# datatypevoid/babble

Hardware: AMD Instinct MI355X
Metric: consensus-ordered events/sec at N=256 peers (1 GPU and 8-GPU batched sims) (higher is better)
Workload: dtype int32

## Files before the change

babble_amd/_lib.py:

```python
from __future__ import annotations

import ctypes as C
import os

import numpy as np

HERE = os.path.dirname(os.path.abspath(__file__))
LIB_PATH = os.path.join(HERE, os.environ.get("HGX_LIB", "libhgx.so"))

_L = None


class HgxError(RuntimeError):

    def __init__(self, code: int, msg: str):
        super().__init__(msg)
        self.code = code
        self.msg = msg


class hgx_error(C.Structure):
    _fields_ = [("code", C.c_int32), ("msg", C.c_char * 252)]


# ... 146 lines not shown
    _sig(L, "hgx_get_block", i32, [p, i32, i32, p, E])
    _sig(L, "hgx_consensus_received", i32, [p, i32, i64, i64, p, p, p])
    _sig(L, "hgx_last_from", i32, [p, i32, p, p, E])
    _sig(L, "hgx_participant_events", i32, [p, i32, i64, p, i64, p, E])
    _sig(L, "hgx_participant_event", i32, [p, i32, i64, p, E])
    _sig(L, "hgx_get_root", i32, [p, i32, p, p, p, p, E])
    _sig(L, "hgx_get_event", i32, [p, i64, p, p, p, p, p, p, p, E])
    _sig(L, "hgx_wire_info", i32, [p, i64, i64, p, p, p])
    _sig(L, "hgx_read_wire_info", i32, [p, i32, i64, i32, i64, p, p, E])
    _sig(L, "hgx_diff_wire", i32, [p, i32, p, i64, p, i64, C.POINTER(C.c_int64), C.POINTER(C.c_int32), E])
    _sig(L, "hgx_keep_bodies", i32, [p, i64, i64, E])
    _sig(L, "hgx_bodies_state", i32, [p, C.POINTER(C.c_int64), C.POINTER(C.c_int64), C.POINTER(C.c_int64)])
    _sig(L, "hgx_get_event_bodies", i32, [p, p, i64, p, p, p, i64, p, i64, C.POINTER(C.c_int64),
                                          C.POINTER(C.c_int64), E])
    _sig(L, "hgx_block_transactions", i32, [p, i32, i64, p, i64, p, i64, C.POINTER(C.c_int64),
                                            C.POINTER(C.c_int64), E])
    _sig(L, "hgx_get_block_hash", i32, [p, i32, i64, p, E])
    _sig(L, "hgx_block_hash_batch", i32, [i32, p, p, p, p, p, i64, p, E])
    _sig(L, "hgx_diff_wire_bodies", i32, [p, i32, p, i64, p, C.POINTER(hgx_wire_body_out), i64, C.POINTER(C.c_int64),
                                          C.POINTER(C.c_int64), C.POINTER(C.c_int64), C.POINTER(C.c_int32), E])
    _sig(L, "hgx_get_rounds", i32, [p, i64, i64, p, p, p])
    _sig(L, "hgx_get_received", i32, [p, i64, i64, p, p])
    _sig(L, "hgx_get_coords", i32, [p, i64, p, p])
    for nm in ("hgx_ancestor", "hgx_self_ancestor", "hgx_see", "hgx_strongly_see", "hgx_round", "hgx_witness"):
        _sig(L, nm, i32, [p, i64, i64] if nm not in ("hgx_round", "hgx_witness") else [p, i64])
    _sig(L, "hgx_oldest_self_ancestor_to_see", i64, [p, i64, i64])
    _sig(L, "hgx_block_hash", i32, [i64, i32, p, p, i32, p])
    _sig(L, "hgx_sha256_batch", i32, [i32, p, p, i64, p, p])
    _sig(L, "hgx_sha256_batch_device", i32, [p, p, i64, p, p])
    _sig(L, "hgx_p256_verify_batch", i32, [i32, p, i32, p, p, p, p, i64, p, p])
    _sig(L, "hgx_p256_verify_bench", i32, [i32, p, i32, p, p, p, p, i64, i32, i32, p, C.POINTER(C.c_double)])
    _sig(L, "hgx_sha256_bench", i32, [i32, i64, i32, i32, C.c_uint64, i32, i32, C.POINTER(C.c_double),
                                      C.POINTER(C.c_int64), C.POINTER(C.c_int64), i64, p])
    _sig(L, "hgx_phase_times", i32, [p, p, i32])
    _sig(L, "hgx_kernel_stats", i32, [p, i32, C.c_char_p, i32, C.POINTER(C.c_double), C.POINTER(C.c_int64),
                                      C.POINTER(C.c_double)])
    _sig(L, "hgx_reset_stats", i32, [p])
    _sig(L, "hgx_set_kernel_timing", i32, [p, i32])
    _sig(L, "hgx_set_coord_storage", i32, [p, i32])
    _sig(L, "hgx_set_fame_tally", i32, [p, i32])
    _sig(L, "hgx_set_round_kernel", i32, [p, i32])
    _sig(L, "hgx_set_sort_kernel", i32, [p, i32])
    _sig(L, "hgx_set_round_shards", i32, [p, i32])
    _sig(L, "hgx_set_shard_remote", i32, [p, i32])
    _sig(L, "hgx_exchange_floor_bench", i32, [i32, i32, i32, i32, C.POINTER(C.c_double)])
    _sig(L, "hgx_seg_sort_check", i32, [i32, i32, p, i32, p, p, p, i32, p, C.POINTER(C.c_int32)])
# ... 32 lines not shown
```

babble_amd/csrc/hgx_api.cpp:

```cpp
#include <algorithm>
#include <array>
#include <chrono>
#include <cstdio>
#include <cstring>
#include <mutex>
#include <tuple>
#include <set>
#include <new>
#include <cstdlib>
#include <string>
#include <thread>
#include <vector>

#include "hgx.h"
#include "hgx_bodies.h"
#include "hgx_bodystore.h"
#include "hgx_diff.h"
#include "hgx_engine.h"
#include "hgx_wire_plan.h"

namespace {

struct Block {
    int32_t rr;
// ... 2691 lines not shown
    }
    return HGX_OK;
}

int32_t hgx_get_received(hgx_ctx* c, int64_t first, int64_t count, int32_t* rr, int64_t* cts) {
    if (!c || first < 0 || count < 0 || first + count > c->E) return HGX_ERR_INVALID;
    DeviceGuard dg(c);
    if (ensure_received(c)) return HGX_ERR_DEVICE;
    for (int64_t k = 0; k < count; k++) {
        const size_t x = (size_t)(first + k);
        const bool have = x < c->rr_cache.size();
        if (rr) rr[k] = have ? c->rr_cache[x] : -1;
        if (cts) cts[k] = (have && c->rr_cache[x] >= 0) ? c->cts_cache[x] : 0;
    }
    return HGX_OK;
}

int32_t hgx_get_coords(hgx_ctx* c, int64_t gid, int32_t* la, int32_t* fd) {
    if (!c || gid < 0 || gid >= c->E_div || !c->divided) return HGX_ERR_INVALID;
    DeviceGuard dg(c);
    return c->eng.get_coords(gid, la, fd) == hipSuccess ? HGX_OK : HGX_ERR_DEVICE;
}

static bool known_div(hgx_ctx* c, int64_t x) { return c && x >= 0 && x < c->E_div && c->divided; }
static bool same_graph(hgx_ctx* c, int64_t x, int64_t y) { return graph_of(c, x) == graph_of(c, y); }

int32_t hgx_ancestor(hgx_ctx* c, int64_t x, int64_t y) {
    if (x == y) return 1;
    if (!known_div(c, x) || !known_div(c, y)) return 0;
    DeviceGuard dg(c);
    if (ensure_mirror(c) || !same_graph(c, x, y)) return 0;
    std::vector<int32_t> la(c->n), fd(c->n);
    if (c->eng.get_coords(x, la.data(), fd.data()) != hipSuccess) return 0;
    return la[c->creator[(size_t)y] % c->n] >= c->index32[(size_t)y] ? 1 : 0;
}
int32_t hgx_self_ancestor(hgx_ctx* c, int64_t x, int64_t y) {
    if (x == y) return 1;
    if (!c || x < 0 || y < 0 || x >= c->E || y >= c->E) return 0;
    DeviceGuard dg(c);
    if (ensure_mirror(c)) return 0;
    return (c->creator[(size_t)x] == c->creator[(size_t)y] && c->index32[(size_t)x] >= c->index32[(size_t)y]) ? 1 : 0;
}
int32_t hgx_see(hgx_ctx* c, int64_t x, int64_t y) { return hgx_ancestor(c, x, y); }
int32_t hgx_strongly_see(hgx_ctx* c, int64_t x, int64_t y) {
    if (!known_div(c, x) || !known_div(c, y)) return 0;
    DeviceGuard dg(c);
// ... 326 lines not shown
```

babble_amd/csrc/hgx_engine.cpp:

```cpp
#include "hgx_engine.h"
#include "hgx_bodystore.h"

#include <algorithm>
#include <array>
#include <chrono>
#include <cstdio>
#include <cstdlib>
#include <cstring>
#include <functional>

namespace hgx {

template <typename T>
hipError_t DBuf<T>::alloc(size_t count) {
    release();
    if (count == 0) count = 1;
    hipError_t e = hipMalloc((void**)&p, count * sizeof(T));
    if (e == hipSuccess) n = count; else p = nullptr;
    return e;
}

template <typename T>
hipError_t DBuf<T>::grow_copy(size_t count, size_t keep, hipStream_t s) {
    if (count <= n) return hipSuccess;
// ... 1297 lines not shown
    HGX_TRY(hipMemcpyAsync(ntx, g_ntx.p + gid, 4, hipMemcpyDeviceToHost, stream));
    HGX_TRY(hipMemcpyAsync(&nil, g_txnil.p + gid, 1, hipMemcpyDeviceToHost, stream));
    HGX_TRY(hipStreamSynchronize(stream));
    *tx_nil = nil;
    return hipSuccess;
}

hipError_t Engine::reserve_rounds(int32_t rounds) {
    rounds = std::max<int32_t>(rounds, 1);
    drop_step_graph();
    Bm.release(); WLA.release(); WFD.release(); wflag.release(); wstat.release(); wcoin.release();
    active.release(); Tthr.release(); fw.release(); elig.release(); ur_empty.release(); Smat.release();
    Vbuf.release(); fame.release(); blk_cnt.release(); blk_loaded.release(); blk_ntx.release(); blk_nil.release();
    ovf.release();
    WLAT.release();
    r_cap = 0;
    R = 0;
    E_div = 0;
    HGX_TRY(ensure_round_cap(rounds));
    return hipStreamSynchronize(stream);
}

int Engine::rebuild_segments(int64_t En, int coord_compact) const {
    if (G != 1 || En < (int64_t)kLaSegMinRows * C) return 1;
    const int cap_segs = (int)std::max<int64_t>(kLaMaxSegs, En / C / (2 * kLaHeadRows));
    return la_segs_override > 0 ? la_segs_override : la_wave_segments(n, coord_compact, num_cus, cap_segs);
}

void Engine::divide_rounds_rows(RoundsHost& out) {
    if (!rows_pending) return;
    rows_pending = false;
    for (size_t k = 0; k < rows_n && k < stage_out.size(); k++) {
        StagedD2H& d = stage_out[k];
        std::memcpy(d.dst, h_stage + d.off, d.bytes);
        d.bytes = 0;
    }
    out.bm.resize((size_t)(R + 1) * C);
    out.wflag.resize((size_t)R * C);
}

int32_t Engine::recv_round_lo(const RoundsHost& rh, int& max_unrecv) const {
    int32_t lo = R;
    max_unrecv = 0;
    if (E_div == 0 || rh.R == 0) return lo;
    for (int c = 0; c < C; c++) {
        const int32_t k = h_fu[c], len = h_len_div[c];
        if (k >= len) continue;
// ... 334 lines not shown

hipError_t Engine::get_coords(int64_t gid, int32_t* la, int32_t* fd) {
    int32_t pos = 0;
    HGX_TRY(hipMemcpyAsync(&pos, g_pos.p + gid, 4, hipMemcpyDeviceToHost, stream));
    HGX_TRY(hipStreamSynchronize(stream));
    if (!compact) {
        HGX_TRY(hipMemcpyAsync(la, LA.p + (size_t)pos * n, (size_t)n * 4, hipMemcpyDeviceToHost, stream));
        HGX_TRY(hipMemcpy2DAsync(fd, 4, FDT.p + pos, (size_t)fd_ld * 4, 4, (size_t)n, hipMemcpyDeviceToHost, stream));
        return hipStreamSynchronize(stream);
    }
    std::vector<uint16_t> l16(n), f16(n);
    const uint16_t* la16 = (const uint16_t*)LA.p;
    const uint16_t* fd16 = (const uint16_t*)FDT.p;
    HGX_TRY(hipMemcpyAsync(l16.data(), la16 + (size_t)pos * n, (size_t)n * 2, hipMemcpyDeviceToHost, stream));
    HGX_TRY(hipMemcpy2DAsync(f16.data(), 2, fd16 + pos, (size_t)fd_ld * 2, 2, (size_t)n, hipMemcpyDeviceToHost, stream));
    HGX_TRY(hipStreamSynchronize(stream));
    for (int i = 0; i < n; i++) {
        la[i] = (int32_t)l16[i] - 1;
        fd[i] = f16[i] == 0xFFFF ? 2147483647 : (int32_t)f16[i];
    }
    return hipSuccess;
}

}


namespace hgx {
void StepGraph::drop() {
    if (exec) (void)hipGraphExecDestroy(exec);
    if (graph) (void)hipGraphDestroy(graph);
    exec = nullptr;
    graph = nullptr;
}

void Engine::drop_step_graph() {
    for (auto& g : step_g) g.drop();
}
}
```

babble_amd/csrc/hgx_engine.h:

```cpp
#pragma once

#include <hip/hip_runtime.h>

#include <cstdint>
#include <string>
#include <atomic>
#include <condition_variable>
#include <mutex>
#include <thread>
#include <vector>

#include "hgx_divide_plan.h"
#include "hgx_ingest_cols.h"
#include "hgx_kernels.h"

#ifndef HGX_TRY
#define HGX_TRY(x)                              \
    do {                                        \
        hipError_t _e = (x);                    \
        if (_e != hipSuccess) return _e;        \
    } while (0)
#endif

namespace hgx {
// ... 223 lines not shown
    hipError_t find_order(const std::vector<uint8_t>& elig, const std::vector<uint8_t>& famous,
                          const std::vector<uint8_t>& ur_empty, int32_t r0, int max_unrecv, OrderHost& out);
    int32_t recv_round_lo(const RoundsHost& rh, int& max_unrecv) const;
    hipError_t find_order_begin(const std::vector<uint8_t>& elig, const std::vector<uint8_t>& famous,
                                const std::vector<uint8_t>& ur_empty, int32_t r0, int max_unrecv, OrderHost& out);
    hipError_t find_order_end(OrderHost& out, int32_t* order_dst = nullptr);
    int64_t shard_values(int lo, int hi) const;
    hipError_t shard_copy(int lo, int hi, void* buf, bool on_device, bool to_buf);
    int shard_lo = 0, shard_hi = 0;
    hipError_t set_roots(const std::vector<int32_t>& round, const std::vector<uint8_t>& y_ext);
    hipError_t set_root_others(const uint8_t* keys32, int64_t count);
    bool others_trust = false;
    bool rooted = false;
    int root_gmax = -1;
    hipError_t round_first_gids(int32_t r0, std::vector<int32_t>& out);
    hipError_t copy_order(int32_t* dst, int64_t first, int64_t count);
    hipError_t sync() { return hipStreamSynchronize(stream); }

    hipError_t reset_received();
    hipError_t reserve_rounds(int32_t rounds);
    hipError_t get_rounds(std::vector<int32_t>& round_by_gid);
    hipError_t get_received(std::vector<int32_t>& rr, std::vector<int64_t>& cts);
    hipError_t get_coords(int64_t gid, int32_t* la, int32_t* fd);

    int n = 0, G = 0, C = 0, sm = 0, nw = 1;
    int64_t cap = 0, E = 0, E_div = 0;
    int64_t Ppos = 0;
    bool incremental = true;
    bool last_rebuild = false;
    int32_t R = 0;
    int la_sweeps = 0;
    int la_kernel = 0;
    bool la_wave_used = false;
    int la_wave_segs = 1;
    int la_segs_override = 0;
    int num_cus = 256;
    static constexpr int kLaMaxSegs = 16;
    static constexpr int kLaHeadRows = 64;
    static constexpr int kLaSegMinRows = 512;
    int64_t la_wave_fallbacks = 0;
    bool la_verified = false;
    bool la_verify_always = false;
    int compact = 0;
    bool force_coord32 = false;
    int64_t la_rows = 0;
    static constexpr int kLaSeg = 16;
// ... 260 lines not shown
```

babble_amd/csrc/hgx_kernels.h:

```cpp
#pragma once

#include <hip/hip_runtime.h>

#include <cstdint>
#include <functional>
#include <vector>

namespace hgx {

constexpr int32_t kMaxI32 = 2147483647;
constexpr int32_t kWlatNotFamous = -2147483647 - 1;
constexpr int kOpkBits = 21;

struct DevArrays {
    const int32_t *g_creator, *g_index, *g_op, *g_ntx;
    const int64_t* g_ts;
    const uint8_t *g_S, *g_coin, *g_loaded, *g_txnil;
    int32_t *g_rr, *g_pos;
    int64_t* g_ck;
    int64_t* g_cts;
    const int32_t *c_off, *c_len, *c_base;
    int32_t *p_gid, *p_chain, *p_op, *p_opu, *p_round, *p_rr;
    int32_t* p_opk;
    int64_t *p_ts, *p_cts;
// ... 144 lines not shown
    int32_t* st[kMaxShards] = {};
    const void* FDT[kMaxShards] = {};
    int32_t c_split[kMaxShards + 1] = {};
};
hipError_t launch_xchg_floor(hipStream_t s, int C, int n, int rounds, uint32_t* rows, uint64_t* gran, int32_t* st);
hipError_t launch_round_p(hipStream_t s, const RoundArgs& A, uint32_t* FD8p, uint64_t* gran, int32_t* status,
                          int32_t* fin, int r0, int r_end, int init, int num_cus, int c_lo = 0, int c_hi = -1,
                          const RoundPWindows* win_dev = nullptr, int nwin = 1);
void launch_round_p_tail(hipStream_t s, const RoundArgs& A, const int32_t* fin, int r_last);
void launch_round_p_post(hipStream_t s, const RoundArgs& A, int r_lo, int r_hi);
bool round_pb_ok(int n, int G);
hipError_t launch_round_pb(hipStream_t s, const RoundArgs& A, uint32_t* FD8p, uint64_t* gran, int32_t* status,
                           int32_t* fin, const int32_t* amap, int na, int r0, int r_end, int num_cus, bool init);
void launch_round_pb_silent(hipStream_t s, const RoundArgs& A, int r_lo, int r_hi);
void launch_root_floor(hipStream_t s, const DevArrays& a, const int32_t* root_round, int32_t* gfl, int32_t* gB,
                       int gmax, int C, int n, int max_len);
void launch_round_first_gid(hipStream_t s, const DevArrays& a, int r0, int R, int C, int32_t* first);
void launch_last_round(hipStream_t s, int rs, int R, int G, int C, int n, const uint8_t* wstat, int32_t* lr);
void step_prof_dump();
void round_k_prof_dump();
void round_p_prof_dump();
void round_pb_prof_dump();
void round_g_prof_dump();
void launch_fame(hipStream_t s, const DevArrays& a, int r0, int R, int C, int n, int nw, int sm, int G, int tally);
void launch_wla_transpose(hipStream_t s, const DevArrays& a, int r0, int R, int G, int C, int n);
void launch_threshold(hipStream_t s, const DevArrays& a, int r0, int R, int C, int n);
void launch_round_received(hipStream_t s, const DevArrays& a, int R, int C, int n, int max_unrecv);
void launch_fu_advance(hipStream_t s, const DevArrays& a, int C);
void launch_fu_count(hipStream_t s, const DevArrays& a, int64_t E);
void launch_cts(hipStream_t s, const DevArrays& a, int c_lo, int c_cnt, int C, int n, int64_t P, int max_cnt);
bool cts_pipe_ok(int n, int C);
bool launch_cts_pipe(hipStream_t s, const DevArrays& a, int c_lo, int c_cnt, int C, int n, int64_t P, int max_cnt);
bool cts_row_ok(int n);
int cts_row_tile();
bool launch_cts_row(hipStream_t s, const DevArrays& a, int c_lo, int c_cnt, int C, int n, int64_t P, int max_cnt,
                    int R, int k_rows);
void launch_cts_shard_copy(hipStream_t s, const DevArrays& a, int lo, int hi, const int32_t* offs, int64_t* buf,
                           int to_buf);
void launch_minmax(hipStream_t s, const DevArrays& a, int32_t m);
void launch_sort(hipStream_t s, const DevArrays& a, int32_t m, int64_t cmin, int cts_bits, int R, int n,
                 int seg_bits, uint32_t** final_vals, uint64_t** final_keys);
int seg_sort_cap();
void launch_seg_count(hipStream_t s, const DevArrays& a, int32_t m, int R, int n, int nseg, uint32_t* segc,
                      unsigned long long* max_out);
hipError_t launch_sort_seg(hipStream_t s, const DevArrays& a, int32_t m, int64_t cmin, int cts_bits, int R, int n, int nseg,
                     uint32_t* segoff, uint32_t* segcur, int max_seg, uint32_t** final_vals, uint64_t** final_keys,
// ... 97 lines not shown
```

babble_amd/csrc/hgx_la_wave.hip:

```cpp
#include <hip/hip_runtime.h>

#include <algorithm>
#include <cstdint>

#include "hgx_device.h"
#include "hgx_kernels.h"

namespace hgx {

namespace {

template <typename CT>
struct LaW;
template <>
struct LaW<int32_t> {
    static constexpr uint32_t kNone = 0xFFFFFFFFu;
    __device__ __forceinline__ static uint32_t wmax(uint32_t a, uint32_t b) {
        return (uint32_t)max((int32_t)a, (int32_t)b);
    }
    static constexpr int kPerWord = 1;
    __device__ __forceinline__ static uint32_t own_mask(int) { return 0xFFFFFFFFu; }
    __device__ __forceinline__ static uint32_t own_bits(int, int32_t own) { return (uint32_t)own; }
};
template <>
struct LaW<uint16_t> {
    static constexpr uint32_t kNone = 0u;
    typedef unsigned short u16x2 __attribute__((ext_vector_type(2)));
    __device__ __forceinline__ static uint32_t wmax(uint32_t a, uint32_t b) {
        const u16x2 m = __builtin_elementwise_max(__builtin_bit_cast(u16x2, a), __builtin_bit_cast(u16x2, b));
        return __builtin_bit_cast(uint32_t, m);
    }
    static constexpr int kPerWord = 2;
    __device__ __forceinline__ static uint32_t own_mask(int cl) { return 0xFFFFu << ((cl & 1) * 16); }
    __device__ __forceinline__ static uint32_t own_bits(int cl, int32_t own) {
        return ((uint32_t)(own + 1) & 0xFFFFu) << ((cl & 1) * 16);
    }
};

#define HGX_CB() asm volatile("" ::: "memory")
__device__ __forceinline__ int32_t lds_ld(const int32_t* p) {
    HGX_CB();
    const int32_t v = *p;
    HGX_CB();
    return v;
}
__device__ __forceinline__ void lds_st(int32_t* p, int32_t v) {
    HGX_CB();
    *p = v;
    HGX_CB();
}

template <int DW>
__device__ __forceinline__ void settle(uint32_t (&v)[DW]) {
#pragma unroll
    for (int w = 0; w < DW; w++) asm volatile("" : "+v"(v[w]));
}

template <int DW>
__device__ __forceinline__ void ring_load(const uint32_t* p, uint32_t (&v)[DW]) {
// ... 16 lines not shown
    HGX_CB();
}
template <int DW>
__device__ __forceinline__ void ring_store(uint32_t* p, const uint32_t (&v)[DW]) {
    HGX_CB();
    if constexpr (DW % 8 == 0) {
#pragma unroll
        for (int k = 0; k < DW / 4; k++) ((uint4*)p)[k] = make_uint4(v[4 * k], v[4 * k + 1], v[4 * k + 2], v[4 * k + 3]);
    } else if constexpr (DW == 4) *(uint4*)p = make_uint4(v[0], v[1], v[2], v[3]);
    else if constexpr (DW == 2) *(uint2*)p = make_uint2(v[0], v[1]);
    else *p = v[0];
    HGX_CB();
}
template <int DW>
__device__ __forceinline__ void row_store(uint32_t* p, const uint32_t (&v)[DW]) {
    if constexpr (DW % 8 == 0) {
#pragma unroll
        for (int k = 0; k < DW / 4; k++) ((uint4*)p)[k] = make_uint4(v[4 * k], v[4 * k + 1], v[4 * k + 2], v[4 * k + 3]);
    } else if constexpr (DW == 4) *(uint4*)p = make_uint4(v[0], v[1], v[2], v[3]);
    else if constexpr (DW == 2) *(uint2*)p = make_uint2(v[0], v[1]);
    else *p = v[0];
}

constexpr int kTagEmpty = -1, kTagBusy = -2;
constexpr int kNoDesc = -2147483647 - 1;
constexpr uint32_t kSpinCap = 1u << 24;

}

__device__ __forceinline__ int chain_lower_bound(const int32_t* __restrict__ p_gid, int off, int len, int64_t x) {
    int lo = 0, hi = len;
    while (lo < hi) {
        const int mid = (lo + hi) >> 1;
        if ((int64_t)p_gid[off + mid] < x) lo = mid + 1;
        else hi = mid;
    }
    return lo;
}

template <typename CT, int DW, int R, int Q, int NLW, int J, int CH, int MODE>
__global__ void __launch_bounds__(1024) k_la_wave(uint32_t* __restrict__ LA, const int32_t* __restrict__ p_opk,
                                                  const int32_t* __restrict__ c_off, const int32_t* __restrict__ c_len,
                                                  const int32_t* __restrict__ c_base,
                                                  const int32_t* __restrict__ c_old,
                                                  const int32_t* __restrict__ p_gid, int64_t E, int nts, int head,
                                                  int n, int lgnp, int nwd, int nblk, int32_t* __restrict__ err,
                                                  const int32_t* __restrict__ lmap, int na, int ts0,
                                                  const int32_t* __restrict__ c_lim,
                                                  const int32_t* __restrict__ gate) {
    typedef LaW<CT> W;
    if (gate && *gate) return;
    extern __shared__ uint32_t smem[];
    const int NP = 1 << lgnp;
    uint32_t* ring_d = smem;
    int32_t* ring_t = (int32_t*)(ring_d + (size_t)R * NP * DW);
    int32_t* q = ring_t + R * NP;
    int32_t* lqv = q + Q * NP;
    int32_t* prog = lqv + n;
    int32_t* s_old = prog + n;
    int32_t* s_off = s_old + n;
    int32_t* s_len = s_off + n;
    int32_t* s_abort = s_len + n;
    const int b = blockIdx.x % nblk, ts = ts0 + (blockIdx.x / nblk) % nts, g = blockIdx.x / nblk / nts;
    const int c0 = g * n;
    const int wb = b * DW;
    const int tid = threadIdx.x;
    for (int t = tid; t < R * NP; t += blockDim.x) ring_t[t] = kTagEmpty;
    for (int t = tid; t < n; t += blockDim.x) {
        const int off = c_off[c0 + t], len = c_len[c0 + t];
        int o = 0, e = len;
        if constexpr (MODE == 1) o = c_old[c0 + t];
        if constexpr (MODE >= 2) {
            const int lim = c_lim ? c_lim[c0 + t] : len;
            o = ts == 0 ? 0 : chain_lower_bound(p_gid, off, lim, E * ts / nts);
            e = ts == nts - 1 ? lim : chain_lower_bound(p_gid, off, lim, E * (ts + 1) / nts);
            if constexpr (MODE == 3) e = ts == 0 ? o : min(e, o + head);
        }
        lqv[t] = o;
        prog[t] = o;
        s_old[t] = o;
        s_off[t] = off;
        s_len[t] = e;
    }
    if (tid == 0) *s_abort = 0;
    __syncthreads();
    const int nl = lmap ? na : n;
    const int ncw = (nl + 63) & ~63;
    if (tid >= ncw) {
        const int l = tid - ncw;
        uint32_t idle = 0;
// ... 2 lines not shown
            int lq[J];
#pragma unroll
            for (int j = 0; j < J; j++) {
                const int i = l + 64 * NLW * j;
                need[j] = false;
                lq[j] = 0;
                if (i < n) {
                    lq[j] = lds_ld(&lqv[i]);
                    if (lq[j] < s_len[i]) {
                        left = true;
                        need[j] = lq[j] + CH <= lds_ld(&prog[i]) + Q;
                    }
                }
            }
            if (!left) break;
            int32_t v[J][CH];
#pragma unroll
            for (int j = 0; j < J; j++)
                if (need[j]) {
                    const int i = l + 64 * NLW * j;
                    const int o = s_off[i] + lq[j], m = s_len[i] - lq[j];
#pragma unroll
                    for (int t = 0; t < CH; t++) v[j][t] = (t < m) ? p_opk[o + t] : -1;
                }
            bool any = false;
#pragma unroll
            for (int j = 0; j < J; j++)
                if (need[j]) {
                    const int i = l + 64 * NLW * j;
#pragma unroll
                    for (int t = 0; t < CH; t++) lds_st(&q[(((unsigned)(lq[j] + t) % Q) << lgnp) + i], v[j][t]);
                    HGX_CB();
                    lds_st(&lqv[i], min(lq[j] + CH, s_len[i]));
                    any = true;
                }
            if (any) {
                idle = 0;
            } else {
                if (lds_ld(s_abort) || ++idle > kSpinCap) break;
                __builtin_amdgcn_s_sleep(1);
            }
        }
        return;
    }
    if (tid >= nl) return;
    const int i = lmap ? lmap[tid] : tid;
    const int len = s_len[i];
    const int off = s_off[i];
    int own0 = c_base[c0 + i];
    asm volatile("" : "+v"(own0));
    const int ow = i / W::kPerWord - wb;
    const uint32_t omask = W::own_mask(i);
    int k = s_old[i];
    uint32_t carry[DW];
#pragma unroll
    for (int w = 0; w < DW; w++)
        carry[w] = (k > 0 && MODE != 2) ? LA[(size_t)(off + k - 1) * nwd + wb + w] : W::kNone;
    settle(carry);
    uint32_t* dst = LA + (size_t)(off + k) * nwd + wb;
    int opv = kNoDesc;
    uint32_t idle = 0;
    while (k < len) {
        const int lv = lds_ld(&lqv[i]);
        const int q0 = lds_ld(&q[(((unsigned)k % Q) << lgnp) + i]);
        const int q1 = lds_ld(&q[(((unsigned)(k + 1) % Q) << lgnp) + i]);
        const bool has_op = opv >= 0;
        const int opc = has_op ? (opv >> kOpkBits) : 0;
        const int opk = has_op ? (opv & ((1 << kOpkBits) - 1)) : 0;
        const int sl = (((unsigned)opk % R) << lgnp) + opc;
        int old = 0;
        int end = 0x7FFFFFFF;
        if constexpr (MODE != 0) old = lds_ld(&s_old[opc]);
        if constexpr (MODE == 3) end = lds_ld(&s_len[opc]);
        const int t1 = lds_ld(&ring_t[sl]);
        uint32_t od[DW];
        ring_load<DW>(ring_d + (size_t)sl * DW, od);
        const int t2 = lds_ld(&ring_t[sl]);
        bool ready = opv == -1 || (has_op && t1 == opk && t2 == opk);
        if (opv == -1) {
#pragma unroll
            for (int w = 0; w < DW; w++) od[w] = W::kNone;
        }
        const bool from_old = MODE != 0 && has_op && (opk < old || opk >= end);
        if (from_old || (has_op && !ready && t1 > opk)) {
            if (MODE == 2 && from_old) {
#pragma unroll
                for (int w = 0; w < DW; w++) od[w] = W::kNone;
            } else {
                uint32_t* src = LA + (size_t)(s_off[opc] + opk) * nwd + wb;
#pragma unroll
                for (int w = 0; w < DW; w++)
                    od[w] = __hip_atomic_load(src + w, __ATOMIC_RELAXED, __HIP_MEMORY_SCOPE_AGENT);
                settle(od);
            }
            ready = true;
        }
        const bool wave_idle = __ballot(ready) == 0;
        if (!ready) {
            if (opv == kNoDesc && lv > k) opv = q0;
            if (wave_idle) __builtin_amdgcn_s_sleep(1);
            if (((++idle) & 4095) == 0 && (idle > kSpinCap || lds_ld(s_abort))) {
                lds_st(s_abort, 1);
                atomicOr(err, 1);
                break;
            }
            continue;
        }
        idle = 0;
        uint32_t v[DW];
#pragma unroll
        for (int w = 0; w < DW; w++) {
            v[w] = W::wmax(carry[w], od[w]);
            v[w] = w == ow ? ((v[w] & ~omask) | W::own_bits(i, own0 + k)) : v[w];
        }
        if constexpr (DW == 16 && R == 8) asm volatile("s_waitcnt vmcnt(23)" ::: "memory");
        else if constexpr (R >= 16) asm volatile("s_waitcnt vmcnt(15)" ::: "memory");
        else asm volatile("s_waitcnt vmcnt(7)" ::: "memory");
        const int ws = (((unsigned)k % R) << lgnp) + i;
        lds_st(&ring_t[ws], kTagBusy);
        ring_store<DW>(ring_d + (size_t)ws * DW, v);
        lds_st(&ring_t[ws], k);
        row_store<DW>(dst, v);
        dst += nwd;
        lds_st(&prog[i], k + 1);
#pragma unroll
        for (int w = 0; w < DW; w++) carry[w] = v[w];
        k++;
        opv = lv > k ? q1 : kNoDesc;
    }
}

namespace {
template <typename CT, int DW, int R, int Q, int NLW, int J, int CH, int MODE>
hipError_t la_wave_launch1(hipStream_t s, const DevArrays& a, int G, int n, const int32_t* c_old, int64_t E, int nts,
                           int head, int32_t* err, const int32_t* lmap, int na, const LaSubset& sub = LaSubset()) {
    const int nwd = a.compact ? n / 2 : n;
    const int nblk = nwd / DW;
    int lgnp = 0;
    while ((1 << lgnp) < n) lgnp++;
    const size_t np2 = (size_t)1 << lgnp;
    const size_t words = np2 * (R * DW + R + Q) + 5 * (size_t)n + 1;
    auto kern = k_la_wave<CT, DW, R, Q, NLW, J, CH, MODE>;
    {
        const hipError_t e = ensure_lds_limit((const void*)kern, 160 * 1024);
        if (e != hipSuccess) return e;
    }
    const int threads = (((lmap ? na : n) + 63) & ~63) + 64 * NLW;
    if (threads > 1024 || (lmap && G != 1)) return hipErrorInvalidValue;
    const int nseg = sub.count > 0 ? sub.count : nts;
    hipLaunchKernelGGL(kern, dim3(G * nseg * nblk), dim3(threads), words * 4, s, (uint32_t*)a.LA, a.p_opk, a.c_off,
                       a.c_len, a.c_base, c_old, a.p_gid, E, nts, head, n, lgnp, nwd, nblk, err, lmap, na, sub.first,
                       sub.c_lim, sub.gate);
    return hipGetLastError();
}
template <typename CT, int DW, int R, int Q, int NLW, int J, int CH>
hipError_t la_wave_launch(hipStream_t s, const DevArrays& a, int G, int n, const int32_t* c_old, int64_t E,
                          int32_t* err, const int32_t* lmap, int na) {
    if (c_old) return la_wave_launch1<CT, DW, R, Q, NLW, J, CH, 1>(s, a, G, n, c_old, E, 1, 0, err, lmap, na);
    return la_wave_launch1<CT, DW, R, Q, NLW, J, CH, 0>(s, a, G, n, nullptr, E, 1, 0, err, lmap, na);
}
struct SegCfg {
    int dw, r, q;
};
inline SegCfg seg_cfg(int n, int nwd) {
// ... 181 lines not shown

hipError_t launch_la_small(hipStream_t s, const DevArrays& a, int G, int n, const int32_t* c_old, size_t lds,
                           int32_t* err) {
    switch (la_small_nw(a.compact ? n / 2 : n)) {
        case 1: return la_small_launch<1>(s, a, G, n, c_old, lds, err);
        case 2: return la_small_launch<2>(s, a, G, n, c_old, lds, err);
        case 4: return la_small_launch<4>(s, a, G, n, c_old, lds, err);
        case 8: return la_small_launch<8>(s, a, G, n, c_old, lds, err);
        case 16: return la_small_launch<16>(s, a, G, n, c_old, lds, err);
        default: return hipErrorInvalidValue;
    }
}

int la_wave_blocks(int n, int compact) {
    const int nwd = compact ? n / 2 : n;
    return nwd / seg_cfg(n, nwd).dw;
}

int la_wave_segments(int n, int compact, int num_cus, int max_segs) {
    const int nwd = compact ? n / 2 : n;
    const SegCfg g = seg_cfg(n, nwd);
    int np2 = 1;
    while (np2 < n) np2 <<= 1;
    const size_t bytes = ((size_t)np2 * (g.r * g.dw + g.r + g.q) + 5 * (size_t)n + 1) * 4;
    const int per_cu = std::max(1, std::min(4, (int)((160 * 1024) / bytes)));
    return std::max(1, std::min(max_segs, per_cu * num_cus / la_wave_blocks(n, compact)));
}

__global__ void __launch_bounds__(256) k_la_seg_bounds(const int32_t* __restrict__ p_gid, const int32_t* __restrict__ c_off,
                                                       const int32_t* __restrict__ c_len, int64_t E, int nts, int n,
                                                       int32_t* __restrict__ tbl) {
    const int t = blockIdx.x;
    for (int c = threadIdx.x; c < n; c += blockDim.x) {
        const int len = c_len[c];
        tbl[(size_t)t * n + c] = t == 0 ? 0 : t == nts ? len : chain_lower_bound(p_gid, c_off[c], len, E * t / nts);
    }
}

template <typename CT>
__global__ void __launch_bounds__(256) k_la_seg_check(const CT* __restrict__ LA, const int32_t* __restrict__ p_gid,
                                                      const int32_t* __restrict__ p_op, const int32_t* __restrict__ p_chain,
                                                      const int32_t* __restrict__ c_off, const int32_t* __restrict__ tbl,
                                                      int64_t E, int nts, int n, int head, int32_t* __restrict__ flag) {
    const int t = 1 + (int)blockIdx.x / n, c = (int)blockIdx.x % n;
    const int o = tbl[(size_t)t * n + c], e = tbl[(size_t)(t + 1) * n + c], off = c_off[c];
    bool bad = false;
    if (e - o > head) {
// ... 52 lines not shown
```

babble_amd/csrc/hgx_rounds.hip:

```cpp
#include <hip/hip_runtime.h>

#include <cstdint>
#include <cstdio>
#include <type_traits>
#include <utility>

#include "hgx_device.h"
#include "hgx_kernels.h"

namespace hgx {

#ifdef HGX_STEP_PROF
__device__ unsigned long long hgx_step_prof[8];
#define HGX_PROF_BEGIN() long long _pt = clock64(); unsigned long long _pa[8] = {0, 0, 0, 0, 0, 0, 0, 0}
#define HGX_PROF(i)                            \
    do {                                       \
        if (threadIdx.x == 0) {                \
            const long long _t = clock64();    \
            _pa[i] += (unsigned long long)(_t - _pt); \
            _pt = _t;                          \
        }                                      \
    } while (0)
#define HGX_PROF_COUNT(i) do { if (threadIdx.x == 0) _pa[i] += 1ull; } while (0)
#define HGX_PROF_END()                                                            \
// ... 638 lines not shown
    if (threadIdx.x == 0) {
        m = max(max(s_max[0], s_max[1]), max(s_max[2], s_max[3]));
        if (m >= 0) atomicMax(&lr[g], m);
    }
}

void launch_last_round(hipStream_t s, int rs, int R, int G, int C, int n, const uint8_t* wstat, int32_t* lr) {
    if (R <= rs) return;
    hipLaunchKernelGGL(k_last_round, dim3(G, (R - rs + 63) / 64), dim3(256), 0, s, rs, R, C, n, wstat, lr);
}


#ifdef HGX_STEP_PROF
void step_prof_dump() {
    unsigned long long h[8];
    if (hipMemcpyFromSymbol(h, HIP_SYMBOL(hgx_step_prof), sizeof(h)) != hipSuccess) return;
    fprintf(stderr, "[hgx] round phases (clk sums; 0 = block-rounds, 6 = wave-0 tallies*1000 + levels):");
    for (int i = 0; i < 8; i++) fprintf(stderr, " %d:%llu", i, h[i]);
    fprintf(stderr, "\n");
    round_k_prof_dump();
    round_p_prof_dump();
    round_pb_prof_dump();
    round_g_prof_dump();
}
#else
void step_prof_dump() {}
#endif

}
```

babble_amd/hashgraph.py:

```python
from __future__ import annotations

import ctypes as C
import os
from typing import List, Optional, Sequence

import numpy as np

from . import _lib
from ._lib import HgxError, hgx_error, hgx_events, ptr

UNKNOWN_PARENT = -2


def compact_columns(t) -> dict:
    ntx = np.where(np.asarray(t.txnil) != 0, -1, np.asarray(t.ntx)).astype(np.int32)
    return dict(creator=np.ascontiguousarray(t.creator, np.int32), index=np.ascontiguousarray(t.index, np.int32),
                sp=np.ascontiguousarray(t.sp, np.int32), op=np.ascontiguousarray(t.op, np.int32),
                ts=np.ascontiguousarray(t.ts, np.int64),
                coin=np.ascontiguousarray(np.asarray(t.hash)[:, 16] != 0, np.uint8),
                s=np.ascontiguousarray(t.s, np.uint8), ntx=ntx)


class HostBuffer:

# ... 766 lines not shown
    def See(self, x: int, y: int) -> bool:
        return bool(self.L.hgx_see(self.ctx, x, y))

    def StronglySee(self, x: int, y: int) -> bool:
        return bool(self.L.hgx_strongly_see(self.ctx, x, y))

    def OldestSelfAncestorToSee(self, x: int, y: int) -> int:
        return int(self.L.hgx_oldest_self_ancestor_to_see(self.ctx, x, y))

    def Round(self, x: int) -> int:
        return int(self.L.hgx_round(self.ctx, x))

    def Witness(self, x: int) -> bool:
        return bool(self.L.hgx_witness(self.ctx, x))

    def coords(self, x: int):
        la = np.zeros(self.n, np.int32)
        fd = np.zeros(self.n, np.int32)
        rc = self.L.hgx_get_coords(self.ctx, x, ptr(la), ptr(fd))
        if rc:
            raise HgxError(rc, "hgx_get_coords failed")
        return la, fd

    def num_events(self) -> int:
        return int(self.L.hgx_num_events(self.ctx))

    def rounds(self):
        E = self.num_events()
        rnd = np.zeros(max(E, 1), np.int32)
        wit = np.zeros(max(E, 1), np.int8)
        fam = np.zeros(max(E, 1), np.int8)
        if E:
            rc = self.L.hgx_get_rounds(self.ctx, 0, E, ptr(rnd), ptr(wit), ptr(fam))
            if rc:
                raise HgxError(rc, "hgx_get_rounds failed")
        return rnd[:E], wit[:E], fam[:E]

    def received(self):
        E = self.num_events()
        rr = np.zeros(max(E, 1), np.int32)
        cts = np.zeros(max(E, 1), np.int64)
        if E:
            rc = self.L.hgx_get_received(self.ctx, 0, E, ptr(rr), ptr(cts))
            if rc:
                raise HgxError(rc, "hgx_get_received failed")
        return rr[:E], cts[:E]
# ... 303 lines not shown
```

include/hgx.h:

```cpp
#ifndef HGX_H
#define HGX_H

#include <stdint.h>

#ifdef __cplusplus
extern "C" {
#endif

#define HGX_ABI_VERSION 6

enum {
    HGX_OK = 0,
    HGX_ERR_KEY_NOT_FOUND = 1,
    HGX_ERR_TOO_LATE = 2,
    HGX_ERR_PASSED_INDEX = 3,
    HGX_ERR_SKIPPED_INDEX = 4,
    HGX_ERR_NO_ROOT = 5,
    HGX_ERR_SELF_PARENT = 100,
    HGX_ERR_OTHER_PARENT = 101,
    HGX_ERR_INVALID = 102,
    HGX_ERR_CAPACITY = 103,
    HGX_ERR_SIGNATURE = 104,
    HGX_ERR_DEVICE = 200,
    HGX_ERR_PANIC = 300
// ... 230 lines not shown
                             int64_t* n_bytes, hgx_error* err);
int32_t hgx_block_transactions(hgx_ctx* ctx, int32_t graph, int64_t b, int64_t* tx_off, int64_t tx_cap,
                               uint8_t* tx_bytes, int64_t bytes_cap, int64_t* n_tx, int64_t* n_bytes, hgx_error* err);
int32_t hgx_get_block_hash(hgx_ctx* ctx, int32_t graph, int64_t b, uint8_t* out32, hgx_error* err);
int32_t hgx_block_hash_batch(int32_t device, const int64_t* round_received, const int32_t* ntx,
                             const int32_t* tx_nil, const int64_t* tx_off, const uint8_t* tx_bytes, int64_t count,
                             uint8_t* out32, hgx_error* err);
typedef struct {
    uint8_t* sig_r;
    int64_t* tx_off;
    int64_t tx_cap;
    uint8_t* tx_bytes;
    int64_t bytes_cap;
} hgx_wire_body_out;
int32_t hgx_diff_wire_bodies(hgx_ctx* ctx, int32_t graph, const int32_t* known, int64_t sync_limit,
                             hgx_wire_out* out, hgx_wire_body_out* body, int64_t cap, int64_t* count, int64_t* n_tx,
                             int64_t* n_bytes, int32_t* over_limit, hgx_error* err);

int32_t hgx_get_rounds(hgx_ctx* ctx, int64_t first, int64_t count, int32_t* round, int8_t* witness,
                       int8_t* famous);
int32_t hgx_get_received(hgx_ctx* ctx, int64_t first, int64_t count, int32_t* round_received,
                         int64_t* consensus_ts);
int32_t hgx_get_coords(hgx_ctx* ctx, int64_t gid, int32_t* last_ancestors, int32_t* first_descendants);

int32_t hgx_ancestor(hgx_ctx* ctx, int64_t x, int64_t y);
int32_t hgx_self_ancestor(hgx_ctx* ctx, int64_t x, int64_t y);
int32_t hgx_see(hgx_ctx* ctx, int64_t x, int64_t y);
int32_t hgx_strongly_see(hgx_ctx* ctx, int64_t x, int64_t y);
int64_t hgx_oldest_self_ancestor_to_see(hgx_ctx* ctx, int64_t x, int64_t y);
int32_t hgx_round(hgx_ctx* ctx, int64_t x);
int32_t hgx_witness(hgx_ctx* ctx, int64_t x);

int32_t hgx_block_hash(int64_t round_received, int32_t ntx, const uint8_t* const* tx, const int64_t* tx_len,
                       int32_t tx_nil, uint8_t* out32);

int32_t hgx_sha256_batch(int32_t device, const uint8_t* data, const int64_t* offsets, int64_t count,
                         uint8_t* out32, hgx_error* err);
int32_t hgx_sha256_batch_device(const uint8_t* d_data, const int64_t* d_offsets, int64_t count,
                                uint8_t* d_out32, void* stream);
int32_t hgx_sha256_bench(int32_t device, int64_t count, int32_t min_len, int32_t max_len, uint64_t seed,
                         int32_t warmup, int32_t iters, double* ms_per_launch, int64_t* total_bytes,
                         int64_t* n_blocks, int64_t n_sample, uint8_t* sample32);

int32_t hgx_exchange_floor_bench(int32_t device, int32_t chains, int32_t n, int32_t rounds, double* us_per_round);

int32_t hgx_seg_sort_check(int32_t device, int32_t nseg, const uint32_t* segoff, int32_t m, const uint64_t* keys,
// ... 47 lines not shown
```

Measured before the change: 288.5 million.

## Streamline LA wave loop: sentinel ring slot, sc1 row reads, mask-free owner merge

Reworks the last-ancestor wave kernel's inner loop. A sentinel ring slot replaces the branch for missing other-parents, and slot indices are now advanced incrementally instead of recomputed with modulos. Owner bits are merged through per-word masks with a wave-uniform guard, and read-backs use vectorised sc1 loads. In MODE 2, stale other-parent entries are filtered at queue fill time. Also adds a bulk coordinate read API, an optional profiler, and an override shortcut for segment count; these add LDS use and inline-asm coupling to the gfx950 ISA.

```diff
diff --git a/babble_amd/_lib.py b/babble_amd/_lib.py
--- a/babble_amd/_lib.py
+++ b/babble_amd/_lib.py
@@ -192,6 +192,7 @@
     _sig(L, "hgx_get_rounds", i32, [p, i64, i64, p, p, p])
     _sig(L, "hgx_get_received", i32, [p, i64, i64, p, p])
     _sig(L, "hgx_get_coords", i32, [p, i64, p, p])
+    _sig(L, "hgx_get_coords_range", i32, [p, i64, i64, p, p])
     for nm in ("hgx_ancestor", "hgx_self_ancestor", "hgx_see", "hgx_strongly_see", "hgx_round", "hgx_witness"):
         _sig(L, nm, i32, [p, i64, i64] if nm not in ("hgx_round", "hgx_witness") else [p, i64])
     _sig(L, "hgx_oldest_self_ancestor_to_see", i64, [p, i64, i64])
diff --git a/babble_amd/csrc/hgx_api.cpp b/babble_amd/csrc/hgx_api.cpp
--- a/babble_amd/csrc/hgx_api.cpp
+++ b/babble_amd/csrc/hgx_api.cpp
@@ -2737,6 +2737,13 @@
     return c->eng.get_coords(gid, la, fd) == hipSuccess ? HGX_OK : HGX_ERR_DEVICE;
 }
 
+int32_t hgx_get_coords_range(hgx_ctx* c, int64_t first, int64_t count, int32_t* la, int32_t* fd) {
+    if (!c || first < 0 || count < 0 || first + count > c->E_div || !c->divided || (count > 0 && (!la || !fd)))
+        return HGX_ERR_INVALID;
+    DeviceGuard dg(c);
+    return c->eng.get_coords_range(first, count, la, fd) == hipSuccess ? HGX_OK : HGX_ERR_DEVICE;
+}
+
 static bool known_div(hgx_ctx* c, int64_t x) { return c && x >= 0 && x < c->E_div && c->divided; }
 static bool same_graph(hgx_ctx* c, int64_t x, int64_t y) { return graph_of(c, x) == graph_of(c, y); }
 
diff --git a/babble_amd/csrc/hgx_engine.cpp b/babble_amd/csrc/hgx_engine.cpp
--- a/babble_amd/csrc/hgx_engine.cpp
+++ b/babble_amd/csrc/hgx_engine.cpp
@@ -1343,7 +1343,9 @@
 }
 
 int Engine::rebuild_segments(int64_t En, int coord_compact) const {
-    if (G != 1 || En < (int64_t)kLaSegMinRows * C) return 1;
+    if (G != 1) return 1;
+    if (la_segs_override > 0) return la_segs_override;
+    if (En < (int64_t)kLaSegMinRows * C) return 1;
     const int cap_segs = (int)std::max<int64_t>(kLaMaxSegs, En / C / (2 * kLaHeadRows));
     return la_segs_override > 0 ? la_segs_override : la_wave_segments(n, coord_compact, num_cus, cap_segs);
 }
@@ -1724,6 +1726,41 @@
     return hipSuccess;
 }
 
+hipError_t Engine::get_coords_range(int64_t first, int64_t count, int32_t* la, int32_t* fd) {
+    if (count <= 0) return hipSuccess;
+    std::vector<int32_t> pos((size_t)count);
+    HGX_TRY(hipMemcpyAsync(pos.data(), g_pos.p + first, (size_t)count * 4, hipMemcpyDeviceToHost, stream));
+    HGX_TRY(hipStreamSynchronize(stream));
+    const size_t hi = (size_t)*std::max_element(pos.begin(), pos.end()) + 1, csz = compact ? 2 : 4;
+    std::vector<uint8_t> lb(hi * n * csz), fb(hi * n * csz);
+    HGX_TRY(hipMemcpyAsync(lb.data(), LA.p, lb.size(), hipMemcpyDeviceToHost, stream));
+    HGX_TRY(hipMemcpy2DAsync(fb.data(), hi * csz, FDT.p, (size_t)fd_ld * csz, hi * csz, (size_t)n, hipMemcpyDeviceToHost,
+                             stream));
+    HGX_TRY(hipStreamSynchronize(stream));
+    for (int64_t x = 0; x < count; x++) {
+        const size_t p = (size_t)pos[(size_t)x];
+        int32_t* lo = la + (size_t)x * n;
+        int32_t* fo = fd + (size_t)x * n;
+        if (compact) {
+            const uint16_t* l16 = (const uint16_t*)lb.data() + p * n;
+            const uint16_t* f16 = (const uint16_t*)fb.data();
+            for (int i = 0; i < n; i++) {
+                lo[i] = (int32_t)l16[i] - 1;
+                const uint16_t f = f16[(size_t)i * hi + p];
+                fo[i] = f == 0xFFFF ? 2147483647 : (int32_t)f;
+            }
+        } else {
+            const int32_t* l32 = (const int32_t*)lb.data() + p * n;
+            const int32_t* f32 = (const int32_t*)fb.data();
+            for (int i = 0; i < n; i++) {
+                lo[i] = l32[i];
+                fo[i] = f32[(size_t)i * hi + p];
+            }
+        }
+    }
+    return hipSuccess;
+}
+
 }
 
 
diff --git a/babble_amd/csrc/hgx_engine.h b/babble_amd/csrc/hgx_engine.h
--- a/babble_amd/csrc/hgx_engine.h
+++ b/babble_amd/csrc/hgx_engine.h
@@ -269,6 +269,7 @@
     hipError_t get_rounds(std::vector<int32_t>& round_by_gid);
     hipError_t get_received(std::vector<int32_t>& rr, std::vector<int64_t>& cts);
     hipError_t get_coords(int64_t gid, int32_t* la, int32_t* fd);
+    hipError_t get_coords_range(int64_t first, int64_t count, int32_t* la, int32_t* fd);
 
     int n = 0, G = 0, C = 0, sm = 0, nw = 1;
     int64_t cap = 0, E = 0, E_div = 0;
diff --git a/babble_amd/csrc/hgx_kernels.h b/babble_amd/csrc/hgx_kernels.h
--- a/babble_amd/csrc/hgx_kernels.h
+++ b/babble_amd/csrc/hgx_kernels.h
@@ -190,6 +190,7 @@
 void round_p_prof_dump();
 void round_pb_prof_dump();
 void round_g_prof_dump();
+void la_wave_prof_dump();
 void launch_fame(hipStream_t s, const DevArrays& a, int r0, int R, int C, int n, int nw, int sm, int G, int tally);
 void launch_wla_transpose(hipStream_t s, const DevArrays& a, int r0, int R, int G, int C, int n);
 void launch_threshold(hipStream_t s, const DevArrays& a, int r0, int R, int C, int n);
diff --git a/babble_amd/csrc/hgx_la_wave.hip b/babble_amd/csrc/hgx_la_wave.hip
--- a/babble_amd/csrc/hgx_la_wave.hip
+++ b/babble_amd/csrc/hgx_la_wave.hip
@@ -2,6 +2,7 @@
 
 #include <algorithm>
 #include <cstdint>
+#include <cstdio>
 
 #include "hgx_device.h"
 #include "hgx_kernels.h"
@@ -21,6 +22,7 @@
     static constexpr int kPerWord = 1;
     __device__ __forceinline__ static uint32_t own_mask(int) { return 0xFFFFFFFFu; }
     __device__ __forceinline__ static uint32_t own_bits(int, int32_t own) { return (uint32_t)own; }
+    __device__ __forceinline__ static uint32_t own_word(uint32_t bits, uint32_t m) { return (bits & m) | ~m; }
 };
 template <>
 struct LaW<uint16_t> {
@@ -35,6 +37,7 @@
     __device__ __forceinline__ static uint32_t own_bits(int cl, int32_t own) {
         return ((uint32_t)(own + 1) & 0xFFFFu) << ((cl & 1) * 16);
     }
+    __device__ __forceinline__ static uint32_t own_word(uint32_t bits, uint32_t m) { return bits & m; }
 };
 
 #define HGX_CB() asm volatile("" ::: "memory")
@@ -97,11 +100,85 @@
     else *p = v[0];
 }
 
+template <int DW>
+__device__ __forceinline__ void row_load_sc1(const uint32_t* p, uint32_t (&v)[DW]) {
+    typedef uint32_t u32x4 __attribute__((ext_vector_type(4)));
+    if constexpr (DW == 16) {
+        u32x4 a, b, c, d;
+        asm volatile(
+            "global_load_dwordx4 %0, %4, off sc1\n\t"
+            "global_load_dwordx4 %1, %4, off offset:16 sc1\n\t"
+            "global_load_dwordx4 %2, %4, off offset:32 sc1\n\t"
+            "global_load_dwordx4 %3, %4, off offset:48 sc1\n\t"
+            "s_waitcnt vmcnt(0)"
+            : "=&v"(a), "=&v"(b), "=&v"(c), "=&v"(d) : "v"(p) : "memory");
+        const u32x4 q4[4] = {a, b, c, d};
+#pragma unroll
+        for (int k = 0; k < 4; k++) { v[4 * k] = q4[k].x; v[4 * k + 1] = q4[k].y; v[4 * k + 2] = q4[k].z; v[4 * k + 3] = q4[k].w; }
+    } else if constexpr (DW == 8) {
+        u32x4 a, b;
+        asm volatile(
+            "global_load_dwordx4 %0, %2, off sc1\n\t"
+            "global_load_dwordx4 %1, %2, off offset:16 sc1\n\t"
+            "s_waitcnt vmcnt(0)"
+            : "=&v"(a), "=&v"(b) : "v"(p) : "memory");
+        v[0] = a.x; v[1] = a.y; v[2] = a.z; v[3] = a.w; v[4] = b.x; v[5] = b.y; v[6] = b.z; v[7] = b.w;
+    } else if constexpr (DW == 4) {
+        u32x4 a;
+        asm volatile(
+            "global_load_dwordx4 %0, %1, off sc1\n\t"
+            "s_waitcnt vmcnt(0)"
+            : "=&v"(a) : "v"(p) : "memory");
+        v[0] = a.x; v[1] = a.y; v[2] = a.z; v[3] = a.w;
+    } else {
+#pragma unroll
+        for (int w = 0; w < DW; w++) v[w] = __hip_atomic_load(p + w, __ATOMIC_RELAXED, __HIP_MEMORY_SCOPE_AGENT);
+#pragma unroll
+        for (int w = 0; w < DW; w++) asm volatile("" : "+v"(v[w]));
+    }
+}
+
 constexpr int kTagEmpty = -1, kTagBusy = -2;
 constexpr int kNoDesc = -2147483647 - 1;
 constexpr uint32_t kSpinCap = 1u << 24;
 
-}
+#ifdef HGX_STEP_PROF
+constexpr int kLaProfWg = 4096, kLaProfN = 6;
+__device__ unsigned long long hgx_la_prof[4][kLaProfWg][kLaProfN];
+#define LA_PROF(...) __VA_ARGS__
+#else
+#define LA_PROF(...)
+#endif
+
+}
+
+#ifdef HGX_STEP_PROF
+void la_wave_prof_dump() {
+    static unsigned long long h[4][kLaProfWg][kLaProfN];
+    if (hipMemcpyFromSymbol(h, HIP_SYMBOL(hgx_la_prof), sizeof(h)) != hipSuccess) return;
+    static const char* const name[kLaProfN] = {"wave trips", "rows", "idle trips", "read-back trips", "read-back lanes",
+                                               "read-back clk"};
+    for (int m = 0; m < 4; m++) {
+        unsigned long long sum[kLaProfN] = {}, mx[kLaProfN] = {};
+        int wgs = 0;
+        for (int g = 0; g < kLaProfWg; g++) {
+            if (!h[m][g][0]) continue;
+            wgs++;
+            for (int x = 0; x < kLaProfN; x++) {
+                sum[x] += h[m][g][x];
+                mx[x] = std::max(mx[x], h[m][g][x]);
+            }
+        }
+        if (!wgs) continue;
+        fprintf(stderr, "[hgx] k_la_wave MODE %d: %d workgroups;", m, wgs);
+        for (int x = 0; x < kLaProfN; x++) fprintf(stderr, " %s %llu (max/wg %llu)%s", name[x], sum[x], mx[x], x + 1 < kLaProfN ? "," : "\n");
+    }
+    void* dp = nullptr;
+    if (hipGetSymbolAddress(&dp, HIP_SYMBOL(hgx_la_prof)) == hipSuccess) (void)hipMemset(dp, 0, sizeof(h));
+}
+#else
+void la_wave_prof_dump() {}
+#endif
 
 __device__ __forceinline__ int chain_lower_bound(const int32_t* __restrict__ p_gid, int off, int len, int64_t x) {
     int lo = 0, hi = len;
@@ -127,9 +204,10 @@
     if (gate && *gate) return;
     extern __shared__ uint32_t smem[];
     const int NP = 1 << lgnp;
+    const int NS = R * NP;
     uint32_t* ring_d = smem;
-    int32_t* ring_t = (int32_t*)(ring_d + (size_t)R * NP * DW);
-    int32_t* q = ring_t + R * NP;
+    int32_t* ring_t = (int32_t*)(ring_d + (size_t)(NS + 1) * DW);
+    int32_t* q = ring_t + NS + 1;
     int32_t* lqv = q + Q * NP;
     int32_t* prog = lqv + n;
     int32_t* s_old = prog + n;
@@ -140,7 +218,9 @@
     const int c0 = g * n;
     const int wb = b * DW;
     const int tid = threadIdx.x;
-    for (int t = tid; t < R * NP; t += blockDim.x) ring_t[t] = kTagEmpty;
+    for (int t = tid; t < NS; t += blockDim.x) ring_t[t] = kTagEmpty;
+    if (tid < DW) ring_d[(size_t)NS * DW + tid] = W::kNone;
+    if (tid == 0) ring_t[NS] = 0;
     for (int t = tid; t < n; t += blockDim.x) {
         const int off = c_off[c0 + t], len = c_len[c0 + t];
         int o = 0, e = len;
@@ -189,6 +269,11 @@
                     const int o = s_off[i] + lq[j], m = s_len[i] - lq[j];
 #pragma unroll
                     for (int t = 0; t < CH; t++) v[j][t] = (t < m) ? p_opk[o + t] : -1;
+                    if constexpr (MODE == 2) {
+#pragma unroll
+                        for (int t = 0; t < CH; t++)
+                            if (v[j][t] >= 0 && (v[j][t] & ((1 << kOpkBits) - 1)) < s_old[v[j][t] >> kOpkBits]) v[j][t] = -1;
+                    }
                 }
             bool any = false;
 #pragma unroll
@@ -217,7 +302,13 @@
     int own0 = c_base[c0 + i];
     asm volatile("" : "+v"(own0));
     const int ow = i / W::kPerWord - wb;
-    const uint32_t omask = W::own_mask(i);
+    const bool wave_owns = __ballot(ow >= 0 && ow < DW) != 0;
+    uint32_t om[DW];
+#pragma unroll
+    for (int w = 0; w < DW; w++) {
+        om[w] = w == ow ? W::own_mask(i) : 0u;
+        asm volatile("" : "+v"(om[w]));
+    }
     int k = s_old[i];
     uint32_t carry[DW];
 #pragma unroll
@@ -227,42 +318,38 @@
     uint32_t* dst = LA + (size_t)(off + k) * nwd + wb;
     int opv = kNoDesc;
     uint32_t idle = 0;
+    int qa = (((unsigned)k % Q) << lgnp) + i, qb = (((unsigned)(k + 1) % Q) << lgnp) + i;
+    int ws = (((unsigned)k % R) << lgnp) + i;
+    LA_PROF(unsigned p_trips = 0, p_rows = 0, p_idle = 0, p_rbt = 0, p_rbl = 0; unsigned long long p_clk = 0;)
     while (k < len) {
         const int lv = lds_ld(&lqv[i]);
-        const int q0 = lds_ld(&q[(((unsigned)k % Q) << lgnp) + i]);
-        const int q1 = lds_ld(&q[(((unsigned)(k + 1) % Q) << lgnp) + i]);
+        const int q0 = lds_ld(&q[qa]);
+        const int q1 = lds_ld(&q[qb]);
         const bool has_op = opv >= 0;
-        const int opc = has_op ? (opv >> kOpkBits) : 0;
-        const int opk = has_op ? (opv & ((1 << kOpkBits) - 1)) : 0;
-        const int sl = (((unsigned)opk % R) << lgnp) + opc;
+        const int opd = has_op ? opv : 0;
+        const int opc = opd >> kOpkBits;
+        const int opk = opd & ((1 << kOpkBits) - 1);
+        const int sl = has_op ? (int)(((unsigned)opk % R) << lgnp) + opc : NS;
         int old = 0;
         int end = 0x7FFFFFFF;
-        if constexpr (MODE != 0) old = lds_ld(&s_old[opc]);
+        if constexpr (MODE == 1 || MODE == 3) old = lds_ld(&s_old[opc]);
         if constexpr (MODE == 3) end = lds_ld(&s_len[opc]);
         const int t1 = lds_ld(&ring_t[sl]);
         uint32_t od[DW];
         ring_load<DW>(ring_d + (size_t)sl * DW, od);
         const int t2 = lds_ld(&ring_t[sl]);
-        bool ready = opv == -1 || (has_op && t1 == opk && t2 == opk);
-        if (opv == -1) {
-#pragma unroll
-            for (int w = 0; w < DW; w++) od[w] = W::kNone;
-        }
-        const bool from_old = MODE != 0 && has_op && (opk < old || opk >= end);
-        if (from_old || (has_op && !ready && t1 > opk)) {
-            if (MODE == 2 && from_old) {
-#pragma unroll
-                for (int w = 0; w < DW; w++) od[w] = W::kNone;
-            } else {
-                uint32_t* src = LA + (size_t)(s_off[opc] + opk) * nwd + wb;
-#pragma unroll
-                for (int w = 0; w < DW; w++)
-                    od[w] = __hip_atomic_load(src + w, __ATOMIC_RELAXED, __HIP_MEMORY_SCOPE_AGENT);
-                settle(od);
-            }
+        bool ready = opv != kNoDesc && t1 == opk && t2 == opk;
+        const bool from_old = (MODE == 1 || MODE == 3) && has_op && (opk < old || opk >= end);
+        const bool back = from_old || (has_op && !ready && t1 > opk);
+        LA_PROF(const bool p_any = __ballot(back) != 0; const unsigned long long p_t0 = __builtin_amdgcn_s_memtime();)
+        if (back) {
+            row_load_sc1<DW>(LA + (size_t)(s_off[opc] + opk) * nwd + wb, od);
             ready = true;
-        }
+            LA_PROF(p_rbl++;)
+        }
+        LA_PROF(p_trips++; if (p_any) { p_rbt++; p_clk += __builtin_amdgcn_s_memtime() - p_t0; })
         const bool wave_idle = __ballot(ready) == 0;
+        LA_PROF(if (wave_idle) p_idle++;)
         if (!ready) {
             if (opv == kNoDesc && lv > k) opv = q0;
             if (wave_idle) __builtin_amdgcn_s_sleep(1);
@@ -276,14 +363,19 @@
         idle = 0;
         uint32_t v[DW];
 #pragma unroll
-        for (int w = 0; w < DW; w++) {
-            v[w] = W::wmax(carry[w], od[w]);
-            v[w] = w == ow ? ((v[w] & ~omask) | W::own_bits(i, own0 + k)) : v[w];
-        }
+        for (int w = 0; w < DW; w++) v[w] = W::wmax(carry[w], od[w]);
+        if (wave_owns) {
+            const uint32_t ob = W::own_bits(i, own0 + k);
+#pragma unroll
+            for (int w = 0; w < DW; w++) v[w] = W::wmax(v[w], W::own_word(ob, om[w]));
+        }
+#ifdef HGX_LA_VMCNT28
+        if constexpr (DW == 16 && R == 8) asm volatile("s_waitcnt vmcnt(28)" ::: "memory");
+#else
         if constexpr (DW == 16 && R == 8) asm volatile("s_waitcnt vmcnt(23)" ::: "memory");
+#endif
         else if constexpr (R >= 16) asm volatile("s_waitcnt vmcnt(15)" ::: "memory");
         else asm volatile("s_waitcnt vmcnt(7)" ::: "memory");
-        const int ws = (((unsigned)k % R) << lgnp) + i;
         lds_st(&ring_t[ws], kTagBusy);
         ring_store<DW>(ring_d + (size_t)ws * DW, v);
         lds_st(&ring_t[ws], k);
@@ -294,7 +386,30 @@
         for (int w = 0; w < DW; w++) carry[w] = v[w];
         k++;
         opv = lv > k ? q1 : kNoDesc;
-    }
+        qa = qb;
+        qb = (qb + NP) & (Q * NP - 1);
+        ws = (ws + NP) & (R * NP - 1);
+        LA_PROF(p_rows++;)
+    }
+#ifdef HGX_STEP_PROF
+    {
+        unsigned (*p_w)[kLaProfN] = (unsigned (*)[kLaProfN])(s_abort + 1);
+        const int wv = tid >> 6;
+        for (int x = 0; x < kLaProfN; x++) p_w[wv][x] = 0;
+        HGX_CB();
+        atomicMax(&p_w[wv][0], p_trips);
+        atomicAdd(&p_w[wv][1], p_rows);
+        atomicMax(&p_w[wv][2], p_idle);
+        atomicMax(&p_w[wv][3], p_rbt);
+        atomicAdd(&p_w[wv][4], p_rbl);
+        atomicMax(&p_w[wv][5], (unsigned)min(p_clk, 0xFFFFFFFFull));
+        HGX_CB();
+        if ((tid & 63) == 0) {
+            const int wg = min((int)blockIdx.x + ts0 * nblk, kLaProfWg - 1);
+            for (int x = 0; x < kLaProfN; x++) atomicAdd(&hgx_la_prof[MODE][wg][x], (unsigned long long)p_w[wv][x]);
+        }
+    }
+#endif
 }
 
 namespace {
@@ -306,7 +421,12 @@
     int lgnp = 0;
     while ((1 << lgnp) < n) lgnp++;
     const size_t np2 = (size_t)1 << lgnp;
-    const size_t words = np2 * (R * DW + R + Q) + 5 * (size_t)n + 1;
+    const size_t words0 = np2 * (R * DW + R + Q) + (DW + 1) + 5 * (size_t)n + 1;
+#ifdef HGX_STEP_PROF
+    const size_t words = words0 + 16 * kLaProfN;
+#else
+    const size_t words = words0;
+#endif
     auto kern = k_la_wave<CT, DW, R, Q, NLW, J, CH, MODE>;
     {
         const hipError_t e = ensure_lds_limit((const void*)kern, 160 * 1024);
@@ -534,7 +654,7 @@
     const SegCfg g = seg_cfg(n, nwd);
     int np2 = 1;
     while (np2 < n) np2 <<= 1;
-    const size_t bytes = ((size_t)np2 * (g.r * g.dw + g.r + g.q) + 5 * (size_t)n + 1) * 4;
+    const size_t bytes = ((size_t)np2 * (g.r * g.dw + g.r + g.q) + (g.dw + 1) + 5 * (size_t)n + 1) * 4;
     const int per_cu = std::max(1, std::min(4, (int)((160 * 1024) / bytes)));
     return std::max(1, std::min(max_segs, per_cu * num_cus / la_wave_blocks(n, compact)));
 }
diff --git a/babble_amd/csrc/hgx_rounds.hip b/babble_amd/csrc/hgx_rounds.hip
--- a/babble_amd/csrc/hgx_rounds.hip
+++ b/babble_amd/csrc/hgx_rounds.hip
@@ -684,6 +684,7 @@
     round_p_prof_dump();
     round_pb_prof_dump();
     round_g_prof_dump();
+    la_wave_prof_dump();
 }
 #else
 void step_prof_dump() {}
diff --git a/babble_amd/hashgraph.py b/babble_amd/hashgraph.py
--- a/babble_amd/hashgraph.py
+++ b/babble_amd/hashgraph.py
@@ -812,6 +812,15 @@
             raise HgxError(rc, "hgx_get_coords failed")
         return la, fd
 
+    def coords_range(self, first: int = 0, count: Optional[int] = None):
+        count = self.num_events() - first if count is None else int(count)
+        la = np.zeros((max(count, 1), self.n), np.int32)
+        fd = np.zeros((max(count, 1), self.n), np.int32)
+        rc = self.L.hgx_get_coords_range(self.ctx, int(first), count, ptr(la), ptr(fd))
+        if rc:
+            raise HgxError(rc, "hgx_get_coords_range failed")
+        return la[:count], fd[:count]
+
     def num_events(self) -> int:
         return int(self.L.hgx_num_events(self.ctx))
 
diff --git a/include/hgx.h b/include/hgx.h
--- a/include/hgx.h
+++ b/include/hgx.h
@@ -276,6 +276,8 @@
 int32_t hgx_get_received(hgx_ctx* ctx, int64_t first, int64_t count, int32_t* round_received,
                          int64_t* consensus_ts);
 int32_t hgx_get_coords(hgx_ctx* ctx, int64_t gid, int32_t* last_ancestors, int32_t* first_descendants);
+int32_t hgx_get_coords_range(hgx_ctx* ctx, int64_t first, int64_t count, int32_t* last_ancestors,
+                             int32_t* first_descendants);
 
 int32_t hgx_ancestor(hgx_ctx* ctx, int64_t x, int64_t y);
 int32_t hgx_self_ancestor(hgx_ctx* ctx, int64_t x, int64_t y);
```

New measurement: 287.6 million. About the same (-0.3%).
